# alonbebchuk/GNN-Pretraining

Hardware: AMD Instinct MI355X
Metric: pretrain graphs/sec (s4 multi-task) (higher is better)
Workload: dtype fp32; 1 GPU; s4 (NFM+LP+NC+GC+GP) pre-training step, 4 domains x 8 synthetic ENZYMES-shaped graphs per rank (input dims 7/4/37/21, hidden 256, 5 GIN layers), PCGrad + clip + AdamW; global_batch_graphs=32, parallelism=dp1, setup_steps=30, full=False, index_rng=reference, index_draws=native (csrc_host/hostdraw.cpp), cross_stream_sync=gates, ranks=1, devices_visible=1

## Files before the change

### gnn_pretraining_amd/_lib.py

```python
from __future__ import annotations

import ctypes as C
import os
import re
from typing import Dict, List

_HERE = os.path.dirname(os.path.abspath(__file__))
LIB_PATH = os.path.join(_HERE, "libgnnmp.so")
HEADER_PATH = os.path.join(os.path.dirname(_HERE), "include", "gnnmp.h")

OK = 0


class GnnmpError(RuntimeError):
    pass


STEP_HEADER_PATH = os.path.join(os.path.dirname(_HERE), "include", "gnnmp_step.h")


def declared_symbols() -> List[str]:
    text = open(HEADER_PATH).read() + open(STEP_HEADER_PATH).read()
    text = re.sub(r"/\*.*?\*/", "", text, flags=re.S)
    return sorted(set(re.findall(r"\b(gmp_[a-z0-9_]+)\s*\(", text)))
# ... 41 lines not shown
                ("sync", C.c_void_p), ("sync_words", C.c_uint32)]


_SIGS: Dict[str, tuple] = {
    "gmp_version": (C.c_int, []),
    "gmp_last_error_string": (C.c_char_p, []),
    "gmp_csr_build_workspace_bytes": (sz, [i64, i64]),
    "gmp_csr_build": (C.c_int, [p, i64, i64, p, p, p, p, p, p, p, p, sz, p]),
    "gmp_csr_build_segmented": (C.c_int, [p, i64, i64, p, p, i32, i64, i64, p, p, p, p, p, p, p, p]),
    "gmp_gin_aggregate_fwd": (C.c_int, [p, p, p, p, p, i64, i32, p]),
    "gmp_gin_aggregate_fwd_rows": (C.c_int, [p, p, p, p, p, i64, i64, i32, p]),
    "gmp_gin_aggregate_bwd_workspace_bytes": (sz, [i64, i32]),
    "gmp_gin_aggregate_bwd": (C.c_int, [p, p, p, p, p, p, p, i64, i32, p, sz, p]),
    "gmp_segment_sum": (C.c_int, [p, p, p, p, i64, i32, i32, i32, p]),
    "gmp_row_gather": (C.c_int, [p, p, p, p, i64, i64, i32, p]),
    "gmp_segment_max_fwd": (C.c_int, [p, p, p, i64, i32, p]),
    "gmp_segment_max_bwd": (C.c_int, [p, p, p, p, p, i64, i32, i32, p]),
    "gmp_gemm_f32_workspace_bytes": (sz, [i32, i64, i64, i64]),
    "gmp_gemm_f32": (C.c_int, [i32, p, p, p, p, i64, i64, i64, i64, i64, i64, f32, i32, i32, p, sz, p]),
    "gmp_gemm_f32_grouped": (C.c_int, [i32, p, p, p, p, i32, p, p, p, p, p, p, i64, i64, i64, i64, i64, i64, f32, i32, i32, p, sz, p]),
    "gmp_gin_aggregate_bwd_ex": (C.c_int, [p, p, p, p, p, p, p, p, i64, i32, p]),
    "gmp_group_sum_1d": (C.c_int, [p, i32, p, p, p, p]),
    "gmp_colsum_workspace_bytes": (sz, [i64, i64]),
    "gmp_colsum": (C.c_int, [p, p, i64, i64, i64, i32, p, sz, p]),
    "gmp_sparse_linear_workspace_bytes": (sz, [i64, i32]),
    "gmp_sparse_linear_fwd": (C.c_int, [p, p, p, i64, i64, p, i64, p, p, i32, i64, p, p, sz, p]),
    "gmp_sparse_linear_wgrad": (C.c_int, [p, p, p, i64, i64, p, i32, p, i64, p, p]),
    "gmp_sparse_csc_workspace_bytes": (sz, [i64, i64, i64]),
    "gmp_sparse_csc_build": (C.c_int, [p, p, p, i64, i64, i64, p, p, p, p, p, sz, p]),
    "gmp_bn_workspace_bytes": (sz, [i64, i32, i32, i64]),
# ... 77 lines not shown
    "gmp_bce_sum_fwd": (C.c_int, [p, p, i64, p, p, sz, p]),
    "gmp_bce_sum_bwd": (C.c_int, [p, p, p, p, i64, p]),
    "gmp_sigmoid_bce_sum_fwd_bwd": (C.c_int, [p, p, i64, p, p, p, p, p, sz, p]),
    "gmp_sigmoid_bce_signed_sum_fwd_bwd": (C.c_int, [p, p, i64, p, p, p, p, p, sz, p]),
    "gmp_cross_entropy_sum_fwd": (C.c_int, [p, p, i64, i32, p, p, sz, p]),
    "gmp_cross_entropy_sum_bwd": (C.c_int, [p, p, i64, i32, p, p, p]),
    "gmp_row_fill": (C.c_int, [p, p, p, i64, i64, i32, i32, p]),
    "gmp_hard_negative_workspace_bytes": (sz, [i64, i64]),
    "gmp_hard_negative_topk": (C.c_int, [p, i64, i64, p, i64, i64, p, p, p, p, sz, p]),
    "gmp_hard_negative_stream_workspace_bytes": (sz, [i64, i64, i64]),
    "gmp_hard_negative_topk_stream": (C.c_int, [p, i64, i64, p, i64, i64, p, p, p, p, sz, p]),
    "gmp_streams_share_queue": (C.c_int, [p, p, p]),
    "gmp_spin_us": (C.c_int, [i32, p]),
    "gmp_gate_wait": (C.c_int, [p, C.c_uint64, i32, p, p]),
    "gmp_gate_open": (C.c_int, [p, i32, p]),
    "gmp_gate_open_by_next_gemm": (C.c_int, [p, i32]),
    "gmp_gate_open_pending": (C.c_int, []),
    "gmp_gate_set_timeout": (C.c_int, [C.c_double]),
    "gmp_counter_add": (C.c_int, [p, C.c_uint64, p]),
    "gmp_aug_workspace_bytes": (sz, [i64, i64, i32]),
    "gmp_aug_node_masks": (C.c_int, [p, p, i32, i64, C.c_uint64, C.c_uint32, p, p]),
    "gmp_aug_node_masks_batch": (C.c_int, [C.POINTER(AugMasksJob), i32, i64, C.c_uint64, p]),
    "gmp_aug_two_views_batch": (C.c_int, [C.POINTER(AugViewsJob), i32, i64, i64, C.c_uint64, p]),
    "gmp_aug_two_views": (C.c_int, [p, p, p, i64, i64, p, i32, i64, i64, i32, C.c_uint64, C.c_uint32, p, p, p, p, p, p, i64, p, p, p, p, p, sz, p]),
    "gmp_aug_negative_edges_workspace_bytes": (sz, [i64, i64, i64]),
    "gmp_aug_negative_edges": (C.c_int, [p, p, p, i64, i64, i32, i64, i64, C.c_uint64, C.c_uint32, p, i64, p, p, p, sz, p]),
    "gmp_aug_negative_edges_batch": (C.c_int, [C.POINTER(AugNegJob), i32, i64, C.c_uint64, p]),
    "gmp_upload": (C.c_int, [i32, p, p, p, p]),
    "gmp_segments_pack": (C.c_int, [p, p, p, i32, i64, p]),
    "gmp_segments_unpack": (C.c_int, [p, p, p, i32, i64, f32, p]),
# ... 40 lines not shown
```

### gnn_pretraining_amd/csrc/pool_gather.hip

```cpp
#include "gnnmp_internal.h"

namespace {

constexpr int BLOCK = 256;
constexpr int WPB = BLOCK / GMP_WAVE;

__device__ __forceinline__ int64_t wave_id() { return ((int64_t)blockIdx.x * BLOCK + threadIdx.x) / GMP_WAVE; }
__device__ __forceinline__ int64_t wave_count() { return (int64_t)gridDim.x * WPB; }

__global__ __launch_bounds__(BLOCK) void row_gather_kernel(const float4* __restrict__ src, const int64_t* __restrict__ idx,
                                                           const int* __restrict__ seg_ptr, float4* __restrict__ out,
                                                           int64_t M, int64_t nsrc, int F4) {
    const int lane = threadIdx.x % GMP_WAVE;
    for (int64_t m = wave_id(); m < M; m += wave_count()) {
        const int64_t r = idx[m];
        const bool ok = r >= 0 && r < nsrc;
        float s = 1.f;
        if (seg_ptr && ok) {
            int c = seg_ptr[r + 1] - seg_ptr[r];
            s = 1.f / (float)(c > 1 ? c : 1);
        }
        for (int c = lane; c < F4; c += GMP_WAVE) {
            float4 v = ok ? src[r * F4 + c] : make_float4(0.f, 0.f, 0.f, 0.f);
            out[m * F4 + c] = make_float4(v.x * s, v.y * s, v.z * s, v.w * s);
        }
    }
}

__global__ __launch_bounds__(BLOCK) void row_gather_scalar_kernel(const float* __restrict__ src, const int64_t* __restrict__ idx,
                                                                  const int* __restrict__ seg_ptr, float* __restrict__ out,
                                                                  int64_t M, int64_t nsrc, int F) {
    const int64_t total = M * F;
    for (int64_t i = (int64_t)blockIdx.x * BLOCK + threadIdx.x; i < total; i += (int64_t)gridDim.x * BLOCK) {
        const int64_t m = i / F, r = idx[m];
        float v = 0.f;
        if (r >= 0 && r < nsrc) {
            v = src[r * F + i % F];
            if (seg_ptr) {
                int c = seg_ptr[r + 1] - seg_ptr[r];
// ... 150 lines not shown
                              int64_t num_src_rows, int feat, gmp_stream_t stream) {
    if (feat <= 0) return gmp::fail(GMP_ERR_ARG, "row_gather: feature width %d", feat);
    if (M < 0 || num_src_rows < 0 || (M > 0 && (!src || !idx || !out))) return gmp::fail(GMP_ERR_ARG, "row_gather: bad argument");
    if (M == 0) return GMP_OK;
    if (feat % 4) {
        int64_t b = (M * feat + BLOCK - 1) / BLOCK;
        hipLaunchKernelGGL(row_gather_scalar_kernel, dim3((unsigned)(b > 4096 ? 4096 : b)), dim3(BLOCK), 0, (hipStream_t)stream, src,
                           idx, seg_ptr, out, M, num_src_rows, feat);
        return gmp::check_launch("row_gather_scalar_kernel");
    }
    hipLaunchKernelGGL(row_gather_kernel, dim3(grid_for(M)), dim3(BLOCK), 0, (hipStream_t)stream, (const float4*)src, idx,
                       seg_ptr, (float4*)out, M, num_src_rows, feat / 4);
    return gmp::check_launch("row_gather_kernel");
}

extern "C" int gmp_segment_max_fwd(const float* x, const int32_t* ptr, float* out, int64_t B, int feat, gmp_stream_t stream) {
    if (int rc = feat_ok("segment_max_fwd", feat)) return rc;
    if (B < 0 || (B > 0 && (!x || !ptr || !out))) return gmp::fail(GMP_ERR_ARG, "segment_max_fwd: bad argument");
    if (B == 0) return GMP_OK;
    hipLaunchKernelGGL(seg_max_fwd_kernel, dim3((unsigned)(B < 65536 ? B : 65536)), dim3(BLOCK), 0, (hipStream_t)stream, (const float4*)x, ptr,
                       (float4*)out, B, feat / 4);
    return gmp::check_launch("seg_max_fwd_kernel");
}

extern "C" int gmp_segment_max_bwd(const float* g_out, const float* x, const float* out, const int32_t* ptr, float* g_x,
                                   int64_t B, int feat, int accumulate, gmp_stream_t stream) {
    if (int rc = feat_ok("segment_max_bwd", feat)) return rc;
    if (B < 0 || (B > 0 && (!g_out || !x || !out || !ptr || !g_x))) return gmp::fail(GMP_ERR_ARG, "segment_max_bwd: bad argument");
    if (B == 0) return GMP_OK;
    hipLaunchKernelGGL(seg_max_bwd_kernel, dim3((unsigned)(B < 65536 ? B : 65536)), dim3(BLOCK), 0, (hipStream_t)stream, (const float4*)g_out,
// ... 25 lines not shown
```

### gnn_pretraining_amd/csrc/step.hip

```cpp
#include "../../include/gnnmp_step.h"
#include <stdlib.h>

#include <atomic>
#include <chrono>
#include <condition_variable>
#include <mutex>
#include <thread>

#include "gnnmp_internal.h"

namespace {

#define GMP_TRY(expr) do { int _rc = (expr); if (_rc != GMP_OK) return _rc; } while (0)


constexpr int H = 256;
constexpr int LAYERS = GMP_STEP_LAYERS, MAXT = GMP_STEP_MAX_TASKS;

struct Dep {
    int flag;
    int ev;
    constexpr uint64_t bit() const { return 1ull << flag; }
};
namespace dep {
constexpr Dep start{0, 0};
constexpr Dep fwd{1, 1};
constexpr Dep main_heads{10, 2};
constexpr Dep l0{35, 3};
constexpr Dep bwd_done{36, 4};
constexpr Dep aux_done{37, 5};
constexpr Dep fwd_fork{39, 6};
constexpr Dep wg1_done{42, -1};
constexpr Dep csr{43, 7};
constexpr Dep lp_csr{44, 8};
constexpr Dep heads_done{-1, 9};
constexpr int EV_HEAD_IN = 10, EV_HEAD_PARAMS = EV_HEAD_IN + MAXT, EV_FWD_JOIN = EV_HEAD_PARAMS + MAXT + 1, EV_LAYER = EV_FWD_JOIN + 2;
constexpr Dep head_in(int ti) { return {2 + ti, EV_HEAD_IN + ti}; }
constexpr Dep head_params(int ti) { return {26 + ti, EV_HEAD_PARAMS + ti}; }
constexpr Dep fwd_join(int k) { return {40 + k, EV_FWD_JOIN + k}; }
constexpr Dep gu_ready(int l) { return {11 + 2 * l, EV_LAYER + 4 * l}; }
constexpr Dep gz1_ready(int l) { return {12 + 2 * l, EV_LAYER + 4 * l + 2}; }
constexpr Dep dw2_done(int l) { return {-1, EV_LAYER + 4 * l + 1}; }
constexpr Dep aux_layer(int l) { return {21 + l, EV_LAYER + 4 * l + 3}; }
}
constexpr int NEV = dep::EV_LAYER + 4 * LAYERS;
constexpr int F_ERR = 63;

struct SyncState {
    int32_t* flags = nullptr;
// ... 32 lines not shown
    c.dropout_p = (dropout && d.training) ? d.dropout_p : 0.f;
    c.seed = d.seed;
    c.stream_id = site;
    c.seed_dev = nullptr;
    return c;
}

int gemm(int mode, const float* A, const float* B, const float* bias, float* C, int64_t M, int64_t N, int64_t K, int64_t lda,
         int64_t ldb, int64_t ldc, bool relu, gmp_stream_t st) {
    return gmp_gemm_f32(mode, A, B, bias, C, M, N, K, lda, ldb, ldc, 1.f, 0, relu ? 1 : 0, nullptr, 0, st);
}

int lp_fused_level() {
    const char* e = getenv("GMP_LP_FUSED");
    return e ? atoi(e) : 1;
}

bool lp_feat_generated(const gmp_step_desc& d, const gmp_task_desc& t) {
    return lp_fused_level() >= 2 && gmp::lp_feat_gemm_applies(d.h[GMP_STEP_LAYERS], d.flat + t.one_off_w0, d.flat + t.one_off_b0, t.lp_y1, t.lp_gy1,
                                                   d.task_grads + t.one_tg_w0, t.gemm_ws, t.lp_K, H);
}

float* drop(const gmp_step_desc& d, float* src, float* dst, int64_t numel, uint32_t site, gmp_stream_t st, int* rc) {
    *rc = GMP_OK;
    if (!d.training || d.dropout_p <= 0.f) return src;
    *rc = gmp_dropout_fwd(src, dst, numel, d.dropout_p, d.seed, site, st);
    return dst;
}

int mlp2_fwd(const gmp_step_desc& d, const gmp_task_desc& t, float** d1_out, gmp_stream_t st) {
// ... 204 lines not shown
}

extern "C" size_t gmp_step_desc_size(void) { return sizeof(gmp_step_desc); }

namespace {

struct Range { int s0, s1; int64_t r0, r1; hipStream_t st; void* ws; };

struct StepCtx {
    const gmp_step_desc& d;
    const hipStream_t main, aux;
    const gmp_stream_t* const task_streams;
    const bool gates;
    const bool lanes, timing;
    const bool defer;
    hipEvent_t* const ev = events();
    const size_t bn_slice;
    SyncState sync;
    Range ranges[3];
    int nranges = 1;
    float* head_d1[MAXT] = {nullptr};
    hipStream_t helper;
    bool main_heads = false;
    hipStream_t wg1;
    void *wg1_ws, *enc_ws;
    size_t wg_ws_bytes, enc_ws_bytes;
    float* gcur;

    StepCtx(const gmp_step_desc& d_, gmp_stream_t main_, const gmp_stream_t* ts, gmp_stream_t aux_, bool lanes_)
        : d(d_), main((hipStream_t)main_), aux((hipStream_t)aux_), task_streams(ts), gates(d_.sync_flags != nullptr), lanes(lanes_),
          timing(phase_timing()), defer(d_.training != 0), bn_slice(gmp_bn_workspace_bytes(d_.N, 2 * H, d_.S, d_.max_seg)),
          helper(main), wg1(aux), gcur(d_.gA) {
        sync.flags = gates ? d.sync_flags : nullptr;
        sync.epoch = d.epoch;
    }
    hipStream_t head_stream(int ti) const { return (hipStream_t)task_streams[ti]; }
    void* slice(int i) const { return (char*)d.bn_ws + bn_slice * (size_t)i; }
    bool two_wg() const { return wg1 != aux; }
    bool eps_on_aux() const { return gates && defer && aux != main; }

    int open(Dep x, hipStream_t s) const { return gmp_gate_open(d.sync_flags + x.flag, d.epoch, s); }
    int record(Dep x, hipStream_t s) const { (void)hipEventRecord(ev[x.ev], s); return GMP_OK; }
    int wait_event(Dep x, hipStream_t s) const { (void)hipStreamWaitEvent(s, ev[x.ev], 0); return GMP_OK; }
    int await_flags(uint64_t mask, hipStream_t s) const { return gmp_gate_wait(d.sync_flags, mask, d.epoch, d.sync_flags + F_ERR, s); }
    int signal(Dep x, hipStream_t s) const { return gates ? (x.flag < 0 ? GMP_OK : open(x, s)) : (x.ev < 0 ? GMP_OK : record(x, s)); }
    int await(Dep x, hipStream_t s) const { return gates ? await_flags(x.bit(), s) : wait_event(x, s); }
    void signal_by_gemm(Dep x, hipStream_t s) const {
        if (!gates) (void)record(x, s);
        else if (gmp::lane_takes(s)) gmp::signal_on_next_gemm(d.sync_flags + x.flag, d.epoch);
    }
    int signal_flush(Dep x, hipStream_t s) const {
        if (!gates || !gmp::lane_takes(s) || !gmp::signal_pending()) return GMP_OK;
        gmp::signal_on_next_gemm(nullptr, 0);
        return open(x, s);
    }
    int signal_csr(Dep x) const { return lanes ? open(x, aux) : record(x, aux); }
    int await_csr(Dep x, hipStream_t s) const { return lanes ? await_flags(x.bit(), s) : wait_event(x, s); }
};

int check_desc(const gmp_step_desc& d) {
    if (d.hidden != H || d.num_tasks < 1 || d.num_tasks > MAXT || d.num_domains < 1 || d.num_domains > GMP_STEP_MAX_DOMAINS || d.N <= 0 || d.S <= 0 ||
// ... 19 lines not shown
    else
        GMP_TRY(gmp_csr_build(d.edge_index, d.N, d.E, d.csr[0], d.csr[1], d.csr[2], d.csr[3], d.csr[4], d.csr[5], d.csr_status, d.csr_ws, d.csr_ws_bytes, c.aux));
    GMP_TRY(c.signal_csr(dep::csr));
    int lp_task = -1;
    for (int ti = 0; ti < d.num_tasks; ++ti)
        if (d.task[ti].kind == GMP_TASK_LP) lp_task = ti;
    if (lp_task >= 0) {
        const gmp_task_desc& t = d.task[lp_task];
        if (d.lp_S > 0)
            GMP_TRY(gmp_csr_build_segmented(t.lp_edges, d.lp_rows_end, t.lp_K, d.lp_seg_ptr, d.lp_seg_eptr, d.lp_S, d.lp_max_seg_rows, d.lp_max_seg_edges,
                                            d.lp_csr[0], d.lp_csr[1], d.lp_csr[2], d.lp_csr[3], d.lp_csr[4], d.lp_csr[5], d.lp_csr_status, c.aux));
        else
            GMP_TRY(gmp_csr_build(t.lp_edges, d.N, t.lp_K, d.lp_csr[0], d.lp_csr[1], d.lp_csr[2], d.lp_csr[3], d.lp_csr[4], d.lp_csr[5], d.lp_csr_status,
                                  d.lp_csr_ws, d.lp_csr_ws_bytes, c.aux));
    }
    return c.signal_csr(dep::lp_csr);
}

int encoders(StepCtx& c) {
    const gmp_step_desc& d = c.d;
    GMP_TRY(gmp_encoder_fwd(d.x_all, d.x_rows, d.N, d.S, d.src_row, d.seg_ptr, d.seg_dom, (const uint64_t*)d.rowmask, d.tiles, d.num_tiles, d.flat,
                            d.num_domains, d.enc_off_w, d.enc_off_b, d.enc_d_in, d.dpad, d.z0, c.main));
    gmp_bn_config bc = bn_cfg(d, true, true, 1);
    GMP_TRY(gmp_bn_fwd(d.z0, nullptr, d.seg_ptr, d.seg_dom, d.S, d.max_seg, d.N, H, d.flat + d.enc_off_gamma0, d.flat + d.enc_off_beta0,
                       c.defer ? nullptr : d.enc_rm, c.defer ? nullptr : d.enc_rv, d.enc_mean, d.enc_rstd, d.h[0], &bc, c.slice(0), c.bn_slice, c.main));
    if (d.nfm_task >= 0 && d.task[d.nfm_task].num_idx > 0) {
        const gmp_task_desc& t = d.task[d.nfm_task];
        GMP_TRY(gmp_row_gather(d.h[0], t.idx, nullptr, t.nfm_target, t.num_idx, d.N, H, c.main));
        GMP_TRY(gmp_row_fill(d.h[0], t.idx, d.flat + d.off_mask_token, t.num_idx, d.N, H, 1, c.main));
    }
    GMP_TRY(c.await_csr(dep::csr, c.main));
    if (c.timing) (void)hipEventRecord(phase_events()[1], c.main);
    return GMP_OK;
}

void select_forward_ranges(StepCtx& c) {
    const gmp_step_desc& d = c.d;
    hipStream_t fwd_streams[3] = {c.main, c.main, c.main};
    int extra = 0;
    for (int ti = 0; ti < d.num_tasks && extra < 2; ++ti) {
        hipStream_t ts = c.head_stream(ti);
        if (ts != c.main && ts != c.aux && ts != fwd_streams[1]) fwd_streams[++extra] = ts;
    }
    c.ranges[0] = Range{0, d.S, 0, d.N, c.main, d.bn_ws};
    int cuts = 0, prev_seg = 0;
    int64_t prev_row = 0;
// ... 3 lines not shown
        ok = d.fwd_cut_seg[k] > prev_seg && d.fwd_cut_seg[k] < d.S && d.fwd_cut_row[k] - prev_row >= 1024 && d.N - d.fwd_cut_row[k] >= 1024;
        prev_seg = d.fwd_cut_seg[k]; prev_row = d.fwd_cut_row[k];
        ++cuts;
    }
    if (!ok || cuts == 0 || cuts > extra) return;
    c.nranges = cuts + 1;
    for (int k = 0; k < c.nranges; ++k)
        c.ranges[k] = Range{k ? d.fwd_cut_seg[k - 1] : 0, k + 1 < c.nranges ? d.fwd_cut_seg[k] : d.S,
                            k ? d.fwd_cut_row[k - 1] : 0, k + 1 < c.nranges ? d.fwd_cut_row[k] : d.N, fwd_streams[k], c.slice(k)};
}

int stacked_forward(StepCtx& c) {
    const gmp_step_desc& d = c.d;
    const bool split = c.nranges > 1;
    if (split) {
        GMP_TRY(c.signal(dep::fwd_fork, c.main));
        for (int k = 1; k < c.nranges; ++k) GMP_TRY(c.await(dep::fwd_fork, c.ranges[k].st));
    }
    for (int l = 0; l < LAYERS; ++l) {
        const gmp_layer_desc& L = d.layer[l];
        for (int k = 0; k < c.nranges; ++k) {
            const Range& R = c.ranges[k];
            const hipStream_t st = R.st;
            const int64_t M = R.r1 - R.r0;
            const int Sk = R.s1 - R.s0;
            const int32_t* sp = d.seg_ptr + R.s0;
            if (split) GMP_TRY(gmp_gin_aggregate_fwd_rows(d.h[l], d.csr[0], d.csr[1], d.flat + L.off_eps, L.a, R.r0, R.r1, H, st));
            else GMP_TRY(gmp_gin_aggregate_fwd(d.h[l], d.csr[0], d.csr[1], d.flat + L.off_eps, L.a, d.N, H, st));
            GMP_TRY(gemm(GMP_GEMM_NT, L.a + R.r0 * H, d.flat + L.off_w1, d.flat + L.off_b1, L.z1 + R.r0 * 2 * H, M, 2 * H, H, H, H, 2 * H, false, st));
            gmp_bn_config bc = bn_cfg(d, true, false, 0);
            GMP_TRY(gmp_bn_fwd(L.z1, nullptr, sp, nullptr, Sk, d.max_seg, d.N, 2 * H, d.flat + L.off_g1, d.flat + L.off_be1, c.defer ? nullptr : L.rm1,
                               c.defer ? nullptr : L.rv1, L.m1 + (size_t)R.s0 * 2 * H, L.s1 + (size_t)R.s0 * 2 * H, L.r1, &bc, R.ws, c.bn_slice, st));
            GMP_TRY(gemm(GMP_GEMM_NT, L.r1 + R.r0 * 2 * H, d.flat + L.off_w2, d.flat + L.off_b2, L.z2 + R.r0 * H, M, H, 2 * H, 2 * H, 2 * H, H, false, st));
            bc = bn_cfg(d, true, true, 10 + l);
            GMP_TRY(gmp_bn_fwd(L.z2, d.h[l], sp, nullptr, Sk, d.max_seg, d.N, H, d.flat + L.off_g2, d.flat + L.off_be2, c.defer ? nullptr : L.rm2,
                               c.defer ? nullptr : L.rv2, L.m2 + (size_t)R.s0 * H, L.s2 + (size_t)R.s0 * H, d.h[l + 1], &bc, R.ws, c.bn_slice, st));
        }
        if (c.timing && l + 1 < LAYERS) (void)hipEventRecord(phase_events()[2 + l], c.main);
    }
    if (split) {
        for (int k = 1; k < c.nranges; ++k) GMP_TRY(c.signal(dep::fwd_join(k - 1), c.ranges[k].st));
        if (c.gates) GMP_TRY(c.await_flags(dep::fwd_join(0).bit() | (c.nranges > 2 ? dep::fwd_join(1).bit() : 0), c.main));
        else for (int k = 1; k < c.nranges; ++k) GMP_TRY(c.wait_event(dep::fwd_join(k - 1), c.main));
    }
    return GMP_OK;
}

int run_head(StepCtx& c, int ti) {
    const gmp_step_desc& d = c.d;
    const hipStream_t ts = c.head_stream(ti);
    if (ts != c.main) GMP_TRY(c.await(dep::fwd, ts));
    if (d.task[ti].kind == GMP_TASK_LP) GMP_TRY(c.await_csr(dep::lp_csr, ts));
    if (c.timing) { (void)hipEventRecord(head_events()[3 * ti], ts); g_head_recorded[3 * ti] = true; g_head_recorded[3 * ti + 2] = false; }
    GMP_TRY(task_head_inputs(d, ti, c.task_streams[ti], &c.head_d1[ti]));
    if (c.timing) { (void)hipEventRecord(head_events()[3 * ti + 1], ts); g_head_recorded[3 * ti + 1] = true; }
    if (ts == c.main) return c.main_heads = true, GMP_OK;
    c.signal_by_gemm(dep::head_in(ti), ts);
    GMP_TRY(task_head_params(d, ti, c.task_streams[ti], c.head_d1[ti]));
    GMP_TRY(c.signal_flush(dep::head_in(ti), ts));
    if (c.timing) { (void)hipEventRecord(head_events()[3 * ti + 2], ts); g_head_recorded[3 * ti + 2] = true; }
    GMP_TRY(c.signal(dep::head_params(ti), ts));
    if (c.gates) c.sync.head_params_mask |= dep::head_params(ti).bit();
    return GMP_OK;
}

int heads(StepCtx& c) {
    const gmp_step_desc& d = c.d;
    const int T = d.num_tasks;
    if (hipMemsetAsync(d.gA, 0, (size_t)d.N * H * sizeof(float), c.main) != hipSuccess) return gmp::fail(GMP_ERR_LAUNCH, "step: memset");
    GMP_TRY(c.signal(dep::fwd, c.main));
    if (c.timing) (void)hipEventRecord(phase_events()[1 + LAYERS], c.main);
    g_head_tasks = T;
    for (int ti = 0; ti < T; ++ti) {
        hipStream_t ts = c.head_stream(ti);
        if (ts != c.main && (c.helper == c.main || ts != c.aux)) c.helper = ts;
    }
    for (int pass = 0; pass < 2; ++pass)
        for (int ti = 0; ti < T; ++ti)
            if ((c.head_stream(ti) == c.main) == (pass == 1)) GMP_TRY(run_head(c, ti));
    if (c.main_heads) {
        if (c.helper != c.main) {
            GMP_TRY(c.signal(dep::main_heads, c.main));
            GMP_TRY(c.await(dep::main_heads, c.helper));
        }
        for (int ti = 0; ti < T; ++ti)
            if (c.head_stream(ti) == c.main) GMP_TRY(task_head_params(d, ti, c.helper, c.head_d1[ti]));
        if (c.helper != c.main) {
            GMP_TRY(c.signal(dep::head_params(MAXT), c.helper));
            if (c.gates) c.sync.head_params_mask |= dep::head_params(MAXT).bit();
        }
    }
    uint64_t mask = 0;
    for (int ti = 0; ti < T; ++ti) {
        if (c.head_stream(ti) == c.main) continue;
        if (c.gates) mask |= dep::head_in(ti).bit();
        else GMP_TRY(c.wait_event(dep::head_in(ti), c.main));
    }
    GMP_TRY(c.gates ? c.await_flags(mask, c.main) : c.wait_event(dep::lp_csr, c.main));
    if (d.dp_exchange) GMP_TRY(c.signal(dep::heads_done, c.main));
    if (c.timing) (void)hipEventRecord(phase_events()[2 + LAYERS], c.main);
    return GMP_OK;
}

void plan_weight_gradients(StepCtx& c) {
    const gmp_step_desc& d = c.d;
    if (c.gates && c.aux != c.main && !d.dp_exchange && d.gemm_ws_bytes >= ((size_t)36 << 20) && wg1_enabled())
        for (int pass = 0; pass < 2 && c.wg1 == c.aux; ++pass)
            for (int ti = 0; ti < d.num_tasks && c.wg1 == c.aux; ++ti) {
                hipStream_t ts = c.head_stream(ti);
                if (ts != c.main && ts != c.aux && (pass == 1 || d.task[ti].kind != GMP_TASK_LP)) c.wg1 = ts;
            }
    const int parts = c.two_wg() ? 2 : 1;
    c.wg_ws_bytes = (d.gemm_ws_bytes / (parts + 1)) & ~(size_t)255;
// ... 111 lines not shown
    if (c.gates) {
        uint64_t mask = c.sync.head_params_mask;
        if (c.aux != c.main) mask |= dep::aux_done.bit();
        if (c.two_wg()) mask |= dep::wg1_done.bit();
        GMP_TRY(c.await_flags(mask, c.main));
    } else if (c.defer) GMP_TRY(c.await(dep::aux_done, c.main));
    if (d.dp_exchange) GMP_TRY(c.signal(dep::bwd_done, c.main));
    if (c.timing) (void)hipEventRecord(phase_events()[GMP_STEP_PHASES], c.main);
    return GMP_OK;
}

int step_body(const gmp_step_desc* dp, gmp_stream_t main_, const gmp_stream_t* task_streams, gmp_stream_t aux_, bool lanes, bool primary) {
    StepCtx c(*dp, main_, task_streams, aux_, lanes);
    if (c.timing) (void)hipEventRecord(phase_events()[0], c.main);
    gmp::signal_on_next_gemm(nullptr, 0);
    GMP_TRY(graph_structure(c));
    GMP_TRY(encoders(c));
    select_forward_ranges(c);
    GMP_TRY(stacked_forward(c));
    GMP_TRY(heads(c));
    plan_weight_gradients(c);
    for (int l = LAYERS - 1; l >= 0; --l) GMP_TRY(backward_layer(c, l));
    GMP_TRY(tail(c));
    if (primary) g_sync = c.sync;
    return GMP_OK;
}

struct LaneJob {
    const gmp_step_desc* d;
    gmp_stream_t main_, aux_;
    const gmp_stream_t* task_streams;
    int device;
};
// ... 131 lines not shown
```

### gnn_pretraining_amd/csrc/streams.hip

```cpp
#include <stdlib.h>

#include <atomic>

#include "gnnmp_internal.h"

namespace {

__global__ void spin_kernel(uint64_t ticks) {
    const uint64_t t0 = wall_clock64();
    for (int i = 0; i < (1 << 22); ++i) {
        if (wall_clock64() - t0 >= ticks) break;
        __builtin_amdgcn_s_sleep(8);
    }
}

constexpr int GATE_FLAGS = 64;
__global__ void gate_wait_kernel(const int* flags, unsigned long long mask, int want, int* err, unsigned long long timeout_ticks) {
    const int lane = threadIdx.x;
    const bool mine = (mask >> lane) & 1ull;
    bool ok = !mine;
    const unsigned long long t0 = wall_clock64();
    for (unsigned i = 1;; ++i) {
        if (!ok) ok = __hip_atomic_load(flags + lane, __ATOMIC_ACQUIRE, __HIP_MEMORY_SCOPE_AGENT) >= want;
        if (__all(ok)) return;
        __builtin_amdgcn_s_sleep(8);
        if ((i & 1023u) == 0 && wall_clock64() - t0 > timeout_ticks) break;
    }
    if (!ok && err) atomicOr(err, 1);
}
__global__ void gate_open_kernel(int* flag, int value) { __hip_atomic_store(flag, value, __ATOMIC_RELEASE, __HIP_MEMORY_SCOPE_AGENT); }

}

static unsigned long long ticks_of(double seconds) {
    if (!(seconds > 0.0)) seconds = 120.0;
    if (seconds > 3600.0) seconds = 3600.0;
    return (unsigned long long)(seconds * 1e8);
}
static std::atomic<unsigned long long>& gate_ticks() {
    static std::atomic<unsigned long long> t{ticks_of(getenv("GMP_GATE_TIMEOUT_S") ? atof(getenv("GMP_GATE_TIMEOUT_S")) : 120.0)};
    return t;
}
extern "C" int gmp_gate_set_timeout(double seconds) {
    if (!(seconds > 0.0) || seconds > 3600.0) return gmp::fail(GMP_ERR_ARG, "gate_set_timeout: %g s not in (0, 3600]", seconds);
    gate_ticks().store(ticks_of(seconds));
    return GMP_OK;
}

extern "C" int gmp_gate_wait(const int32_t* flags, uint64_t mask, int want, int32_t* err, gmp_stream_t st) {
    if (!flags) return gmp::fail(GMP_ERR_ARG, "gate_wait: null flags");
    if (!mask) return GMP_OK;
    const unsigned long long ticks = gate_ticks().load();
    hipLaunchKernelGGL(gate_wait_kernel, dim3(1), dim3(GATE_FLAGS), 0, (hipStream_t)st, (const int*)flags, (unsigned long long)mask, want, (int*)err, ticks);
    return gmp::check_launch("gate_wait_kernel");
}
extern "C" int gmp_gate_open(int32_t* flag, int value, gmp_stream_t st) {
    if (!flag) return gmp::fail(GMP_ERR_ARG, "gate_open: null flag");
    hipLaunchKernelGGL(gate_open_kernel, dim3(1), dim3(1), 0, (hipStream_t)st, (int*)flag, value);
    return gmp::check_launch("gate_open_kernel");
}

extern "C" int gmp_spin_us(int us, gmp_stream_t st) {
    if (us < 0 || us > 100000) return gmp::fail(GMP_ERR_ARG, "spin_us: %d us not in [0, 100000]", us);
    hipLaunchKernelGGL(spin_kernel, dim3(1), dim3(64), 0, (hipStream_t)st, (uint64_t)us * 100);
    return gmp::check_launch("spin_kernel");
}

extern "C" int gmp_streams_share_queue(gmp_stream_t a_, gmp_stream_t b_, int* share) {
    if (!share) return gmp::fail(GMP_ERR_ARG, "streams_share_queue: null result pointer");
// ... 39 lines not shown
```

### include/gnnmp.h

```cpp
#ifndef GNNMP_H
#define GNNMP_H

#include <stddef.h>
#include <stdint.h>

#ifdef __cplusplus
extern "C" {
#endif

#define GMP_OK 0
#define GMP_ERR_ARG (-1)
#define GMP_ERR_LAUNCH (-2)
#define GMP_ERR_WORKSPACE (-3)
#define GMP_ERR_UNSUPPORTED (-4)

typedef void* gmp_stream_t;

int gmp_version(void);
const char* gmp_last_error_string(void);

size_t gmp_csr_build_workspace_bytes(int64_t num_nodes, int64_t num_edges);
int gmp_csr_build(const int64_t* edge_index, int64_t num_nodes, int64_t num_edges,
                  int32_t* rowptr, int32_t* col, int32_t* perm,
                  int32_t* rowptr_t, int32_t* col_t, int32_t* perm_t,
// ... 12 lines not shown
int gmp_gin_aggregate_bwd(const float* g_out, const int32_t* rowptr_t, const int32_t* col_t, const float* eps,
                          const float* x, float* g_x, float* g_eps, int64_t num_nodes, int feat,
                          void* workspace, size_t workspace_bytes, gmp_stream_t stream);

int gmp_gin_aggregate_bwd_ex(const float* g_out, const int32_t* rowptr_t, const int32_t* col_t, const float* eps,
                             const float* x, const float* addend, float* g_x, float* rowdot, int64_t num_nodes,
                             int feat, gmp_stream_t stream);
int gmp_group_sum_1d(const float* vals, int groups, const int32_t* group_rows_host, const int64_t* out_off_host,
                     float* out, gmp_stream_t stream);

int gmp_segment_sum(const float* src, const int32_t* ptr, const int32_t* idx, float* out,
                    int64_t num_segments, int feat, int mean, int accumulate, gmp_stream_t stream);

int gmp_row_gather(const float* src, const int64_t* idx, const int32_t* seg_ptr, float* out,
                   int64_t num_out_rows, int64_t num_src_rows, int feat, gmp_stream_t stream);

int gmp_segment_max_fwd(const float* x, const int32_t* ptr, float* out, int64_t num_segments, int feat,
                        gmp_stream_t stream);
int gmp_segment_max_bwd(const float* g_out, const float* x, const float* out, const int32_t* ptr,
                        float* g_x, int64_t num_segments, int feat, int accumulate, gmp_stream_t stream);

#define GMP_GEMM_NT 0
#define GMP_GEMM_NN 1
#define GMP_GEMM_TN 2
size_t gmp_gemm_f32_workspace_bytes(int mode, int64_t M, int64_t N, int64_t K);
int gmp_gemm_f32(int mode, const float* A, const float* B, const float* bias, float* C,
                 int64_t M, int64_t N, int64_t K, int64_t lda, int64_t ldb, int64_t ldc,
                 float alpha, int accumulate, int relu, void* workspace, size_t workspace_bytes,
                 gmp_stream_t stream);
int gmp_gemm_f32_grouped(int mode, const float* A, const float* B, const float* bias, float* C, int groups,
// ... 220 lines not shown
size_t gmp_hard_negative_stream_workspace_bytes(int64_t n, int64_t dim, int64_t E);
int gmp_hard_negative_topk_stream(const float* emb, int64_t n, int64_t dim, const int64_t* existing_edges, int64_t E,
                                  int64_t k, int64_t* out_edges, float* out_scores, float* scores_out,
                                  void* workspace, size_t workspace_bytes, gmp_stream_t stream);

int gmp_segments_pack(const float* base, float* packed, const int64_t* table_dev, int n, int64_t total, gmp_stream_t stream);
int gmp_segments_unpack(float* base, const float* packed, const int64_t* table_dev, int n, int64_t total, float scale,
                        gmp_stream_t stream);

int gmp_upload(int n, const void* const* src_pinned_host, void* const* dst, const int64_t* bytes, gmp_stream_t stream);

int gmp_streams_share_queue(gmp_stream_t a, gmp_stream_t b, int* share_host);
int gmp_spin_us(int microseconds, gmp_stream_t stream);
int gmp_gate_wait(const int32_t* flags, uint64_t mask, int want, int32_t* err, gmp_stream_t stream);
int gmp_gate_open(int32_t* flag, int value, gmp_stream_t stream);
int gmp_gate_open_by_next_gemm(int32_t* flag, int value);
int gmp_gate_open_pending(void);
int gmp_gate_set_timeout(double seconds);
int gmp_counter_add(uint64_t* word, uint64_t inc, gmp_stream_t stream);

int gmp_encoder_fwd(const float* x_all, int64_t num_x_rows, int64_t num_rows, int num_segments, const int32_t* src_row, const int32_t* seg_ptr, const int32_t* seg_dom,
                    const uint64_t* row_colmask, const int32_t* tiles, int num_tiles, const float* params,
                    int num_domains, const int64_t* w_off_host, const int64_t* b_off_host,
                    const int32_t* d_in_host, int dpad, float* z, gmp_stream_t stream);
int gmp_encoder_bwd(const float* x_all, int64_t num_x_rows, int64_t num_rows, int num_segments, const int32_t* src_row, const int32_t* seg_ptr, const int32_t* seg_dom,
                    const uint64_t* row_colmask, const float* g_z, int num_domains, const int32_t* d_in_host,
                    int dpad, int groups, const int32_t* group_seg_host, const int64_t* off_w_host,
                    const int64_t* off_b_host, float* grad_out, void* workspace, size_t workspace_bytes,
                    gmp_stream_t stream);

// ... 102 lines not shown
```

Measured before the change: 24270 graphs/s.

## Fuse gate signal/wait launches and move gA zeroing onto aux stream

Adds a combined gate kernel that can open one flag, wait on a mask, then open another flag, so that separate signal and wait launches collapse into one. It also merges the NFM row gather and mask-token fill into a single kernel, and moves the gA memset from the main stream to the aux stream behind a new ga_zero gate. Forward-range selection now happens before graph_structure so the aux path knows whether the split is active. The aim is fewer tiny launches and less serialized work on the main stream in a launch-bound step. The cost is more complex cross-stream dependency logic, where a wrong mask could cause hangs or races.

```diff
diff --git a/gnn_pretraining_amd/_lib.py b/gnn_pretraining_amd/_lib.py
--- a/gnn_pretraining_amd/_lib.py
+++ b/gnn_pretraining_amd/_lib.py
@@ -79,6 +79,7 @@
     "gmp_gin_aggregate_bwd": (C.c_int, [p, p, p, p, p, p, p, i64, i32, p, sz, p]),
     "gmp_segment_sum": (C.c_int, [p, p, p, p, i64, i32, i32, i32, p]),
     "gmp_row_gather": (C.c_int, [p, p, p, p, i64, i64, i32, p]),
+    "gmp_row_gather_fill": (C.c_int, [p, p, p, p, i64, i64, i32, p]),
     "gmp_segment_max_fwd": (C.c_int, [p, p, p, i64, i32, p]),
     "gmp_segment_max_bwd": (C.c_int, [p, p, p, p, p, i64, i32, i32, p]),
     "gmp_gemm_f32_workspace_bytes": (sz, [i32, i64, i64, i64]),
@@ -186,6 +187,7 @@
     "gmp_spin_us": (C.c_int, [i32, p]),
     "gmp_gate_wait": (C.c_int, [p, C.c_uint64, i32, p, p]),
     "gmp_gate_open": (C.c_int, [p, i32, p]),
+    "gmp_gate_wait_ex": (C.c_int, [p, C.c_uint64, i32, p, p, p, p]),
     "gmp_gate_open_by_next_gemm": (C.c_int, [p, i32]),
     "gmp_gate_open_pending": (C.c_int, []),
     "gmp_gate_set_timeout": (C.c_int, [C.c_double]),
diff --git a/gnn_pretraining_amd/csrc/pool_gather.hip b/gnn_pretraining_amd/csrc/pool_gather.hip
--- a/gnn_pretraining_amd/csrc/pool_gather.hip
+++ b/gnn_pretraining_amd/csrc/pool_gather.hip
@@ -23,6 +23,20 @@
         for (int c = lane; c < F4; c += GMP_WAVE) {
             float4 v = ok ? src[r * F4 + c] : make_float4(0.f, 0.f, 0.f, 0.f);
             out[m * F4 + c] = make_float4(v.x * s, v.y * s, v.z * s, v.w * s);
+        }
+    }
+}
+
+__global__ __launch_bounds__(BLOCK) void row_gather_fill_kernel(float4* __restrict__ rows, const int64_t* __restrict__ idx,
+                                                                const float4* __restrict__ token, float4* __restrict__ out,
+                                                                int64_t M, int64_t nrows, int F4) {
+    const int lane = threadIdx.x % GMP_WAVE;
+    for (int64_t m = wave_id(); m < M; m += wave_count()) {
+        const int64_t r = idx[m];
+        const bool ok = r >= 0 && r < nrows;
+        for (int c = lane; c < F4; c += GMP_WAVE) {
+            out[m * F4 + c] = ok ? rows[r * F4 + c] : make_float4(0.f, 0.f, 0.f, 0.f);
+            if (ok) rows[r * F4 + c] = token[c];
         }
     }
 }
@@ -203,6 +217,16 @@
     return gmp::check_launch("row_gather_kernel");
 }
 
+extern "C" int gmp_row_gather_fill(float* rows, const int64_t* idx, const float* token, float* out, int64_t M, int64_t num_rows, int feat,
+                                   gmp_stream_t stream) {
+    if (int rc = feat_ok("row_gather_fill", feat)) return rc;
+    if (M < 0 || num_rows < 0 || (M > 0 && (!rows || !idx || !token || !out))) return gmp::fail(GMP_ERR_ARG, "row_gather_fill: bad argument");
+    if (M == 0) return GMP_OK;
+    hipLaunchKernelGGL(row_gather_fill_kernel, dim3(grid_for(M)), dim3(BLOCK), 0, (hipStream_t)stream, (float4*)rows, idx, (const float4*)token,
+                       (float4*)out, M, num_rows, feat / 4);
+    return gmp::check_launch("row_gather_fill_kernel");
+}
+
 extern "C" int gmp_segment_max_fwd(const float* x, const int32_t* ptr, float* out, int64_t B, int feat, gmp_stream_t stream) {
     if (int rc = feat_ok("segment_max_fwd", feat)) return rc;
     if (B < 0 || (B > 0 && (!x || !ptr || !out))) return gmp::fail(GMP_ERR_ARG, "segment_max_fwd: bad argument");
diff --git a/gnn_pretraining_amd/csrc/step.hip b/gnn_pretraining_amd/csrc/step.hip
--- a/gnn_pretraining_amd/csrc/step.hip
+++ b/gnn_pretraining_amd/csrc/step.hip
@@ -33,6 +33,7 @@
 constexpr Dep wg1_done{42, -1};
 constexpr Dep csr{43, 7};
 constexpr Dep lp_csr{44, 8};
+constexpr Dep ga_zero{45, -1};
 constexpr Dep heads_done{-1, 9};
 constexpr int EV_HEAD_IN = 10, EV_HEAD_PARAMS = EV_HEAD_IN + MAXT, EV_FWD_JOIN = EV_HEAD_PARAMS + MAXT + 1, EV_LAYER = EV_FWD_JOIN + 2;
 constexpr Dep head_in(int ti) { return {2 + ti, EV_HEAD_IN + ti}; }
@@ -95,6 +96,11 @@
 int lp_fused_level() {
     const char* e = getenv("GMP_LP_FUSED");
     return e ? atoi(e) : 1;
+}
+
+bool handoff_enabled() {
+    const char* e = getenv("GMP_STEP_HANDOFF");
+    return !e || atoi(e) != 0;
 }
 
 bool lp_feat_generated(const gmp_step_desc& d, const gmp_task_desc& t) {
@@ -329,11 +335,13 @@
     const bool gates;
     const bool lanes, timing;
     const bool defer;
+    const bool handoff = handoff_enabled();
     hipEvent_t* const ev = events();
     const size_t bn_slice;
     SyncState sync;
     Range ranges[3];
     int nranges = 1;
+    bool fork_fused = false;
     float* head_d1[MAXT] = {nullptr};
     hipStream_t helper;
     bool main_heads = false;
@@ -360,6 +368,10 @@
     int await_flags(uint64_t mask, hipStream_t s) const { return gmp_gate_wait(d.sync_flags, mask, d.epoch, d.sync_flags + F_ERR, s); }
     int signal(Dep x, hipStream_t s) const { return gates ? (x.flag < 0 ? GMP_OK : open(x, s)) : (x.ev < 0 ? GMP_OK : record(x, s)); }
     int await(Dep x, hipStream_t s) const { return gates ? await_flags(x.bit(), s) : wait_event(x, s); }
+    int hand_over(uint64_t mask, int pre, int post, hipStream_t s) const {
+        return gmp_gate_wait_ex(d.sync_flags, mask, d.epoch, d.sync_flags + F_ERR, pre < 0 ? nullptr : d.sync_flags + pre, post < 0 ? nullptr : d.sync_flags + post, s);
+    }
+    bool ga_on_aux() const { return handoff && gates && nranges > 1 && aux != main; }
     void signal_by_gemm(Dep x, hipStream_t s) const {
         if (!gates) (void)record(x, s);
         else if (gmp::lane_takes(s)) gmp::signal_on_next_gemm(d.sync_flags + x.flag, d.epoch);
@@ -409,7 +421,14 @@
             GMP_TRY(gmp_csr_build(t.lp_edges, d.N, t.lp_K, d.lp_csr[0], d.lp_csr[1], d.lp_csr[2], d.lp_csr[3], d.lp_csr[4], d.lp_csr[5], d.lp_csr_status,
                                   d.lp_csr_ws, d.lp_csr_ws_bytes, c.aux));
     }
-    return c.signal_csr(dep::lp_csr);
+    if (!c.ga_on_aux()) return c.signal_csr(dep::lp_csr);
+    if (c.lanes) GMP_TRY(c.hand_over(dep::fwd_fork.bit(), dep::lp_csr.flag, -1, c.aux));
+    else {
+        GMP_TRY(c.signal_csr(dep::lp_csr));
+        GMP_TRY(c.await_flags(dep::fwd_fork.bit(), c.aux));
+    }
+    if (hipMemsetAsync(d.gA, 0, (size_t)d.N * H * sizeof(float), c.aux) != hipSuccess) return gmp::fail(GMP_ERR_LAUNCH, "step: memset");
+    return c.open(dep::ga_zero, c.aux);
 }
 
 int encoders(StepCtx& c) {
@@ -421,10 +440,16 @@
                        c.defer ? nullptr : d.enc_rm, c.defer ? nullptr : d.enc_rv, d.enc_mean, d.enc_rstd, d.h[0], &bc, c.slice(0), c.bn_slice, c.main));
     if (d.nfm_task >= 0 && d.task[d.nfm_task].num_idx > 0) {
         const gmp_task_desc& t = d.task[d.nfm_task];
-        GMP_TRY(gmp_row_gather(d.h[0], t.idx, nullptr, t.nfm_target, t.num_idx, d.N, H, c.main));
-        GMP_TRY(gmp_row_fill(d.h[0], t.idx, d.flat + d.off_mask_token, t.num_idx, d.N, H, 1, c.main));
-    }
-    GMP_TRY(c.await_csr(dep::csr, c.main));
+        if (c.handoff) {
+            GMP_TRY(gmp_row_gather_fill(d.h[0], t.idx, d.flat + d.off_mask_token, t.nfm_target, t.num_idx, d.N, H, c.main));
+        } else {
+            GMP_TRY(gmp_row_gather(d.h[0], t.idx, nullptr, t.nfm_target, t.num_idx, d.N, H, c.main));
+            GMP_TRY(gmp_row_fill(d.h[0], t.idx, d.flat + d.off_mask_token, t.num_idx, d.N, H, 1, c.main));
+        }
+    }
+    c.fork_fused = c.handoff && c.lanes && c.nranges > 1;
+    if (c.fork_fused) GMP_TRY(c.hand_over(dep::csr.bit(), -1, dep::fwd_fork.flag, c.main));
+    else GMP_TRY(c.await_csr(dep::csr, c.main));
     if (c.timing) (void)hipEventRecord(phase_events()[1], c.main);
     return GMP_OK;
 }
@@ -458,7 +483,7 @@
     const gmp_step_desc& d = c.d;
     const bool split = c.nranges > 1;
     if (split) {
-        GMP_TRY(c.signal(dep::fwd_fork, c.main));
+        if (!c.fork_fused) GMP_TRY(c.signal(dep::fwd_fork, c.main));
         for (int k = 1; k < c.nranges; ++k) GMP_TRY(c.await(dep::fwd_fork, c.ranges[k].st));
     }
     for (int l = 0; l < LAYERS; ++l) {
@@ -484,7 +509,9 @@
     }
     if (split) {
         for (int k = 1; k < c.nranges; ++k) GMP_TRY(c.signal(dep::fwd_join(k - 1), c.ranges[k].st));
-        if (c.gates) GMP_TRY(c.await_flags(dep::fwd_join(0).bit() | (c.nranges > 2 ? dep::fwd_join(1).bit() : 0), c.main));
+        const uint64_t joins = dep::fwd_join(0).bit() | (c.nranges > 2 ? dep::fwd_join(1).bit() : 0);
+        if (c.ga_on_aux()) GMP_TRY(c.hand_over(joins | dep::ga_zero.bit(), -1, dep::fwd.flag, c.main));
+        else if (c.gates) GMP_TRY(c.await_flags(joins, c.main));
         else for (int k = 1; k < c.nranges; ++k) GMP_TRY(c.wait_event(dep::fwd_join(k - 1), c.main));
     }
     return GMP_OK;
@@ -493,8 +520,16 @@
 int run_head(StepCtx& c, int ti) {
     const gmp_step_desc& d = c.d;
     const hipStream_t ts = c.head_stream(ti);
-    if (ts != c.main) GMP_TRY(c.await(dep::fwd, ts));
-    if (d.task[ti].kind == GMP_TASK_LP) GMP_TRY(c.await_csr(dep::lp_csr, ts));
+    const bool lp = d.task[ti].kind == GMP_TASK_LP;
+    if (c.handoff && c.gates) {
+        uint64_t mask = ts != c.main ? dep::fwd.bit() | (c.ga_on_aux() ? dep::ga_zero.bit() : 0) : 0;
+        if (lp && c.lanes) mask |= dep::lp_csr.bit();
+        GMP_TRY(c.await_flags(mask, ts));
+        if (lp && !c.lanes) GMP_TRY(c.await_csr(dep::lp_csr, ts));
+    } else {
+        if (ts != c.main) GMP_TRY(c.await(dep::fwd, ts));
+        if (lp) GMP_TRY(c.await_csr(dep::lp_csr, ts));
+    }
     if (c.timing) { (void)hipEventRecord(head_events()[3 * ti], ts); g_head_recorded[3 * ti] = true; g_head_recorded[3 * ti + 2] = false; }
     GMP_TRY(task_head_inputs(d, ti, c.task_streams[ti], &c.head_d1[ti]));
     if (c.timing) { (void)hipEventRecord(head_events()[3 * ti + 1], ts); g_head_recorded[3 * ti + 1] = true; }
@@ -511,8 +546,10 @@
 int heads(StepCtx& c) {
     const gmp_step_desc& d = c.d;
     const int T = d.num_tasks;
-    if (hipMemsetAsync(d.gA, 0, (size_t)d.N * H * sizeof(float), c.main) != hipSuccess) return gmp::fail(GMP_ERR_LAUNCH, "step: memset");
-    GMP_TRY(c.signal(dep::fwd, c.main));
+    if (!c.ga_on_aux()) {
+        if (hipMemsetAsync(d.gA, 0, (size_t)d.N * H * sizeof(float), c.main) != hipSuccess) return gmp::fail(GMP_ERR_LAUNCH, "step: memset");
+        GMP_TRY(c.signal(dep::fwd, c.main));
+    }
     if (c.timing) (void)hipEventRecord(phase_events()[1 + LAYERS], c.main);
     g_head_tasks = T;
     for (int ti = 0; ti < T; ++ti) {
@@ -522,9 +559,15 @@
     for (int pass = 0; pass < 2; ++pass)
         for (int ti = 0; ti < T; ++ti)
             if ((c.head_stream(ti) == c.main) == (pass == 1)) GMP_TRY(run_head(c, ti));
+    uint64_t mask = 0;
+    if (c.gates)
+        for (int ti = 0; ti < T; ++ti)
+            if (c.head_stream(ti) != c.main) mask |= dep::head_in(ti).bit();
+    const bool join_fused = c.handoff && c.gates && c.main_heads && c.helper != c.main;
     if (c.main_heads) {
         if (c.helper != c.main) {
-            GMP_TRY(c.signal(dep::main_heads, c.main));
+            if (join_fused) GMP_TRY(c.hand_over(mask, dep::main_heads.flag, -1, c.main));
+            else GMP_TRY(c.signal(dep::main_heads, c.main));
             GMP_TRY(c.await(dep::main_heads, c.helper));
         }
         for (int ti = 0; ti < T; ++ti)
@@ -534,13 +577,11 @@
             if (c.gates) c.sync.head_params_mask |= dep::head_params(MAXT).bit();
         }
     }
-    uint64_t mask = 0;
-    for (int ti = 0; ti < T; ++ti) {
-        if (c.head_stream(ti) == c.main) continue;
-        if (c.gates) mask |= dep::head_in(ti).bit();
-        else GMP_TRY(c.wait_event(dep::head_in(ti), c.main));
-    }
-    GMP_TRY(c.gates ? c.await_flags(mask, c.main) : c.wait_event(dep::lp_csr, c.main));
+    if (!c.gates) {
+        for (int ti = 0; ti < T; ++ti)
+            if (c.head_stream(ti) != c.main) GMP_TRY(c.wait_event(dep::head_in(ti), c.main));
+        GMP_TRY(c.wait_event(dep::lp_csr, c.main));
+    } else if (!join_fused) GMP_TRY(c.await_flags(mask, c.main));
     if (d.dp_exchange) GMP_TRY(c.signal(dep::heads_done, c.main));
     if (c.timing) (void)hipEventRecord(phase_events()[2 + LAYERS], c.main);
     return GMP_OK;
@@ -682,9 +723,9 @@
     StepCtx c(*dp, main_, task_streams, aux_, lanes);
     if (c.timing) (void)hipEventRecord(phase_events()[0], c.main);
     gmp::signal_on_next_gemm(nullptr, 0);
+    select_forward_ranges(c);
     GMP_TRY(graph_structure(c));
     GMP_TRY(encoders(c));
-    select_forward_ranges(c);
     GMP_TRY(stacked_forward(c));
     GMP_TRY(heads(c));
     plan_weight_gradients(c);
diff --git a/gnn_pretraining_amd/csrc/streams.hip b/gnn_pretraining_amd/csrc/streams.hip
--- a/gnn_pretraining_amd/csrc/streams.hip
+++ b/gnn_pretraining_amd/csrc/streams.hip
@@ -15,20 +15,30 @@
 }
 
 constexpr int GATE_FLAGS = 64;
-__global__ void gate_wait_kernel(const int* flags, unsigned long long mask, int want, int* err, unsigned long long timeout_ticks) {
+__device__ __forceinline__ bool gate_poll(const int* flags, unsigned long long mask, int want, int* err, unsigned long long timeout_ticks) {
     const int lane = threadIdx.x;
     const bool mine = (mask >> lane) & 1ull;
     bool ok = !mine;
     const unsigned long long t0 = wall_clock64();
     for (unsigned i = 1;; ++i) {
         if (!ok) ok = __hip_atomic_load(flags + lane, __ATOMIC_ACQUIRE, __HIP_MEMORY_SCOPE_AGENT) >= want;
-        if (__all(ok)) return;
+        if (__all(ok)) return true;
         __builtin_amdgcn_s_sleep(8);
         if ((i & 1023u) == 0 && wall_clock64() - t0 > timeout_ticks) break;
     }
     if (!ok && err) atomicOr(err, 1);
+    return false;
+}
+__global__ void gate_wait_kernel(const int* flags, unsigned long long mask, int want, int* err, unsigned long long timeout_ticks) {
+    (void)gate_poll(flags, mask, want, err, timeout_ticks);
 }
 __global__ void gate_open_kernel(int* flag, int value) { __hip_atomic_store(flag, value, __ATOMIC_RELEASE, __HIP_MEMORY_SCOPE_AGENT); }
+
+__global__ void gate_ex_kernel(const int* flags, unsigned long long mask, int want, int* err, unsigned long long timeout_ticks, int* pre, int* post) {
+    if (pre && threadIdx.x == 0) __hip_atomic_store(pre, want, __ATOMIC_RELEASE, __HIP_MEMORY_SCOPE_AGENT);
+    if (mask && !gate_poll(flags, mask, want, err, timeout_ticks)) return;
+    if (post && threadIdx.x == 0) __hip_atomic_store(post, want, __ATOMIC_RELEASE, __HIP_MEMORY_SCOPE_AGENT);
+}
 
 }
 
@@ -53,6 +63,14 @@
     const unsigned long long ticks = gate_ticks().load();
     hipLaunchKernelGGL(gate_wait_kernel, dim3(1), dim3(GATE_FLAGS), 0, (hipStream_t)st, (const int*)flags, (unsigned long long)mask, want, (int*)err, ticks);
     return gmp::check_launch("gate_wait_kernel");
+}
+extern "C" int gmp_gate_wait_ex(const int32_t* flags, uint64_t mask, int want, int32_t* err, int32_t* pre_flag, int32_t* post_flag, gmp_stream_t st) {
+    if (mask && !flags) return gmp::fail(GMP_ERR_ARG, "gate_wait_ex: null flags");
+    if (!mask && !pre_flag && !post_flag) return GMP_OK;
+    const unsigned long long ticks = gate_ticks().load();
+    hipLaunchKernelGGL(gate_ex_kernel, dim3(1), dim3(GATE_FLAGS), 0, (hipStream_t)st, (const int*)flags, (unsigned long long)mask, want, (int*)err, ticks,
+                       (int*)pre_flag, (int*)post_flag);
+    return gmp::check_launch("gate_ex_kernel");
 }
 extern "C" int gmp_gate_open(int32_t* flag, int value, gmp_stream_t st) {
     if (!flag) return gmp::fail(GMP_ERR_ARG, "gate_open: null flag");
diff --git a/include/gnnmp.h b/include/gnnmp.h
--- a/include/gnnmp.h
+++ b/include/gnnmp.h
@@ -50,6 +50,8 @@
 
 int gmp_row_gather(const float* src, const int64_t* idx, const int32_t* seg_ptr, float* out,
                    int64_t num_out_rows, int64_t num_src_rows, int feat, gmp_stream_t stream);
+int gmp_row_gather_fill(float* rows, const int64_t* idx, const float* token, float* out, int64_t num_idx, int64_t num_rows, int feat,
+                        gmp_stream_t stream);
 
 int gmp_segment_max_fwd(const float* x, const int32_t* ptr, float* out, int64_t num_segments, int feat,
                         gmp_stream_t stream);
@@ -300,6 +302,7 @@
 int gmp_spin_us(int microseconds, gmp_stream_t stream);
 int gmp_gate_wait(const int32_t* flags, uint64_t mask, int want, int32_t* err, gmp_stream_t stream);
 int gmp_gate_open(int32_t* flag, int value, gmp_stream_t stream);
+int gmp_gate_wait_ex(const int32_t* flags, uint64_t mask, int want, int32_t* err, int32_t* pre_flag, int32_t* post_flag, gmp_stream_t stream);
 int gmp_gate_open_by_next_gemm(int32_t* flag, int value);
 int gmp_gate_open_pending(void);
 int gmp_gate_set_timeout(double seconds);
```

New measurement: 24430 graphs/s (median of 6 runs). About the same (+0.7%).
